# augustgw/early-exit-transformer

Hardware: AMD Instinct MI355X
Metric: mel-frames/sec encoder forward (all exits) + summed per-exit CTC loss, d_model=256 12-layer (higher is better)
Workload: dtype fp16x3 (hi/lo-split fp16 MFMA operands, three products per GEMM, fp32 accumulate; v_mfma_f32_16x16x32_f16); 1 GPU; early_conformer ctc 12-layer d_model=256 (6 exits x 2), batch 64/GPU, mel [80 x 1027] -> T'=256, log-normal synthetic mel, random-init weights (BASELINE.json configs[1]); global_batch=64, mel_frames=1027, parallelism=dp1 (utterance-batch shards), precision_mode=f16x3

## Files before the change

### early_exit_transformer_amd/csrc/ctc.hip

```cpp
#include <limits.h>

#include "eec_kernels.h"

namespace eec {

constexpr int kCtcPerLane = 8;
constexpr int kCtcEmpty = -(1 << 20);
constexpr float kCtcTiny = 7.52316385e-37f;
constexpr float kCtcRedo = -1.f;
__host__ __device__ inline int ctc_watch_slack(int Tq) {
  int lg = 0;
  while (((long long)Tq * 2048) >> lg) ++lg;
  return 120 - 26 - lg;
}

#define EEC_DPP_F(old, src, ctrl) \
  __builtin_bit_cast(float, __builtin_amdgcn_update_dpp(__builtin_bit_cast(int, (float)(old)), __builtin_bit_cast(int, (float)(src)), ctrl, 0xf, 0xf, false))
#define EEC_DPP_I(old, src, ctrl) __builtin_amdgcn_update_dpp((int)(old), (int)(src), ctrl, 0xf, 0xf, false)

__device__ __forceinline__ size_t ctc_store_index(int lat, int Tq, int P, int t, int k, int lane) {
  return (((size_t)lat * Tq + t) * (P + 1) + k) * 64 + lane;
}

template <int P, bool STORE>
__global__ __launch_bounds__(64) void ctc_alpha_kernel(const float* __restrict__ logp, const long long* __restrict__ targets,
                                                       const long long* __restrict__ target_len, int B, int Tq, int V,
                                                       int S, int blank, float* __restrict__ nll, float* __restrict__ astore) {
  const int lat = blockIdx.x, b = lat % B, lane = threadIdx.x;
  const float* lp = logp + (size_t)lat * Tq * V;
  const long long len_raw = target_len[b];
  bool bad = len_raw < 0 || len_raw > (long long)S;
  const int len = bad ? 0 : (int)len_raw;
  const int L = 2 * len + 1;
  int label[P];
  bool skip_ok[P], live[P];
#pragma unroll
  for (int i = 0; i < P; ++i) {
    const int s = lane * P + i;
    label[i] = blank;
    skip_ok[i] = false;
    live[i] = s < L;
    if (s < L && (s & 1)) {
      const int k = s >> 1;
      const long long lab = targets[(size_t)b * S + k];
      if (lab < 0 || lab >= (long long)V) bad = true;
      label[i] = (lab < 0 || lab >= (long long)V) ? blank : (int)lab;
      skip_ok[i] = k > 0 && lab != targets[(size_t)b * S + k - 1];
    }
  }
  bad = __any((int)bad) != 0;
  float livef[P];
#pragma unroll
  for (int i = 0; i < P; ++i) {
    livef[i] = live[i] ? 1.f : 0.f;
    asm volatile("" : "+v"(label[i]));
  }
  float alpha[P], lim[P];
  int ex = kCtcEmpty;
  static_assert(P % 2 == 0, "a lane's first state must be a blank");
  int eloss = kCtcEmpty;
#pragma unroll
  for (int i = 0; i < P; ++i) {
    const int s = lane * P + i;
    const float l0 = lp[label[i]];
    alpha[i] = (s < 2 && s < L) ? __expf(l0) : 0.f;
    eloss = ((s < 2 && s < L) & (l0 > -INFINITY) & (alpha[i] < kCtcTiny)) ? 0 : eloss;
    lim[i] = live[i] ? -INFINITY : INFINITY;
  }
  if (lane == 0) ex = 0;
  auto store = [&](int t) {
    if constexpr (STORE) {
#pragma unroll
      for (int i = 0; i < P; ++i) astore[ctc_store_index(lat, Tq, P, t, i, lane)] = alpha[i];
      astore[ctc_store_index(lat, Tq, P, t, P, lane)] = __builtin_bit_cast(float, ex);
    }
  };
  store(0);
  constexpr int kCtcAhead = P <= 4 ? 16 : 8;
  float emit[kCtcAhead][P];
#pragma unroll
  for (int d = 0; d < kCtcAhead; ++d)
#pragma unroll
    for (int i = 0; i < P; ++i) emit[d][i] = lp[(size_t)min(1 + d, Tq - 1) * V + label[i]];
  auto step = [&](const float (&em)[P], bool renorm) {
    float up1 = EEC_DPP_F(0.f, alpha[P - 1], 0x138);
    float up2 = EEC_DPP_F(0.f, alpha[P - 2], 0x138);
    const int ex_up = EEC_DPP_I(ex, ex, 0x138);
    const int ec = max(ex, ex_up);
    const int d_own = max(ex - ec, -200), d_up = max(ex_up - ec, -200);
    const float up1s = ldexpf(up1, d_up), up2s = ldexpf(up2, d_up);
    bool lost = (up1 > 0.f) & (up1s < kCtcTiny);
    up1 = up1s;
    up2 = up2s;
    float cur[P];
#pragma unroll
    for (int i = 0; i < P; ++i) {
      cur[i] = ldexpf(alpha[i], d_own);
      lost |= (alpha[i] > 0.f) & (cur[i] < kCtcTiny);
    }
    ex = ec;
#pragma unroll
    for (int i = 0; i < P; ++i) {
      const float p1 = i >= 1 ? cur[i - 1] : up1;
      const float p2 = i >= 2 ? cur[i - 2] : (i == 1 ? up1 : up2);
      const float sum = cur[i] + p1 + (skip_ok[i] ? p2 : 0.f);
      alpha[i] = sum * (__expf(em[i]) * livef[i]);
      lost |= (sum > 0.f) & (alpha[i] < kCtcTiny) & (em[i] > lim[i]);
    }
    eloss = lost ? max(eloss, ec) : eloss;
    if (renorm) {
      float m = alpha[0];
#pragma unroll
      for (int i = 1; i < P; ++i) m = fmaxf(m, alpha[i]);
      const bool any = m > 0.f;
      const int e = any ? (int)((__builtin_bit_cast(unsigned, m) >> 23) & 0xffu) - 127 : 0;
#pragma unroll
      for (int i = 0; i < P; ++i) alpha[i] = ldexpf(alpha[i], -e);
      ex = any ? ex + e : kCtcEmpty;
    }
  };
  int t0 = 1;
  for (; t0 + kCtcAhead <= Tq; t0 += kCtcAhead) {
#pragma unroll
    for (int d = 0; d < kCtcAhead; ++d) {
      step(emit[d], (d & 1) != 0);
      store(t0 + d);
      const int tn = min(t0 + d + kCtcAhead, Tq - 1);
#pragma unroll
      for (int i = 0; i < P; ++i) emit[d][i] = lp[(size_t)tn * V + label[i]];
    }
  }
#pragma unroll
  for (int d = 0; d < kCtcAhead; ++d)
    if (t0 + d < Tq) {
      step(emit[d], (d & 1) != 0);
      store(t0 + d);
    }
  float tail = 0.f;
#pragma unroll
  for (int i = 0; i < P; ++i) {
    const int s = lane * P + i;
    if (s == L - 1 || s == L - 2) tail += alpha[i];
  }
  bad = bad || __any((int)(tail != tail)) != 0;
  const int e_lane = tail > 0.f ? ex : kCtcEmpty;
  const int e_max = (int)wave_max((float)e_lane);
  const float total = wave_sum(tail > 0.f ? ldexpf(tail, max(e_lane - e_max, -200)) : 0.f);
  const int e_tot = total > 0.f ? e_max + (int)((__builtin_bit_cast(unsigned, total) >> 23) & 0xffu) - 127 : 2 * kCtcEmpty;
  const bool redo = __any((int)(eloss > kCtcEmpty && eloss > e_tot + ctc_watch_slack(Tq))) != 0;
  if (lane == 0)
    nll[lat] = (bad || total != total) ? __builtin_nanf("")
               : redo                  ? -INFINITY
               : (total > 0.f)         ? -(logf(total) + (float)e_max * 0.6931471805599453f)
                                       : INFINITY;
  if constexpr (STORE) {
    if (lane == 0) {
      float* pinfo = astore + ctc_store_index(gridDim.x, Tq, P, 0, 0, 0) + 2 * (size_t)lat;
      pinfo[0] = (bad || total != total) ? __builtin_nanf("") : redo ? kCtcRedo : total;
      pinfo[1] = __builtin_bit_cast(float, e_max);
    }
  }
}

template <int P>
__global__ __launch_bounds__(64) void ctc_beta_kernel(const float* __restrict__ logp, const long long* __restrict__ targets,
                                                      const long long* __restrict__ target_len, int B, int Tq, int V,
                                                      int S, int blank, const float* __restrict__ nll, float* __restrict__ astore) {
  const int lat = blockIdx.x, b = lat % B, lane = threadIdx.x;
  const float* lp = logp + (size_t)lat * Tq * V;
  float* pinfo = astore + ctc_store_index(gridDim.x, Tq, P, 0, 0, 0) + 2 * (size_t)lat;
  if (pinfo[0] < 0.f) return;
  const long long len_raw = target_len[b];
  const int len = (len_raw < 0 || len_raw > (long long)S) ? 0 : (int)len_raw;
  const int L = 2 * len + 1;
  int label[P];
  bool skip_ok[P];
  float livef[P], lim[P];
  bool redo = false;
#pragma unroll
  for (int i = 0; i < P; ++i) {
    const int s = lane * P + i;
    label[i] = blank;
    skip_ok[i] = false;
    livef[i] = s < L ? 1.f : 0.f;
    lim[i] = s < L ? -INFINITY : INFINITY;
    if (s < L && (s & 1)) {
      const int k = s >> 1;
      const long long lab = targets[(size_t)b * S + k];
      label[i] = (lab < 0 || lab >= (long long)V) ? blank : (int)lab;
      skip_ok[i] = k > 0 && lab != targets[(size_t)b * S + k - 1];
    }
    asm volatile("" : "+v"(label[i]));
  }
  bool skip_dn[P];
  {
    const int n0 = EEC_DPP_I(0, (int)skip_ok[0], 0x130), n1 = EEC_DPP_I(0, (int)skip_ok[1], 0x130);
#pragma unroll
    for (int i = 0; i < P; ++i) skip_dn[i] = i + 2 < P ? skip_ok[i + 2] : ((i + 2 - P == 0 ? n0 : n1) != 0);
  }
  const float ptot = pinfo[0];
  const bool usable = ptot > 0.f && ptot < INFINITY;
  const int ishift = usable ? -__builtin_bit_cast(int, pinfo[1]) : 0;
  const float fscale = usable ? 1.0f / ptot : 0.f;
  const int e_ptot = (int)((__builtin_bit_cast(unsigned, ptot) >> 23) & 0xffu) - 127;
  const int e_harm = usable ? -ishift + e_ptot + ctc_watch_slack(Tq) : INT_MAX;
  const int sh_harm = 120 - 26 - 2 + e_ptot;
  float beta[P];
  int eb = kCtcEmpty;
  bool any0 = false;
#pragma unroll
  for (int i = 0; i < P; ++i) {
    const int s = lane * P + i;
    beta[i] = (s < L && (s == L - 1 || s == L - 2)) ? 1.f : 0.f;
    any0 = any0 || beta[i] != 0.f;
  }
  if (any0) eb = 0;
  constexpr int kAhead = P <= 4 ? 8 : 4;
  float emit[kAhead][P], al[kAhead][P + 1];
  auto fetch = [&](int slot, int t) {
    const int tc = max(t, 0);
#pragma unroll
    for (int i = 0; i < P; ++i) emit[slot][i] = lp[(size_t)tc * V + label[i]];
#pragma unroll
    for (int k = 0; k <= P; ++k) al[slot][k] = astore[ctc_store_index(lat, Tq, P, tc, k, lane)];
  };
#pragma unroll
  for (int d = 0; d < kAhead; ++d) fetch(d, Tq - 1 - d);
  auto step = [&](int slot, int t, bool renorm) {
    const int ea = __builtin_bit_cast(int, al[slot][P]);
    const int sh = max(min(ea + eb + ishift, 126), -300);
#pragma unroll
    for (int i = 0; i < P; ++i) {
      const float ab = al[slot][i] * beta[i];
      redo |= (al[slot][i] > 0.f) & (beta[i] > 0.f) & (ab < kCtcTiny) & (sh > sh_harm);
      astore[ctc_store_index(lat, Tq, P, t, i, lane)] = ldexpf(ab * fscale, sh) * livef[i];
    }
    float bw[P];
    bool lost = false;
#pragma unroll
    for (int i = 0; i < P; ++i) {
      bw[i] = beta[i] * (__expf(emit[slot][i]) * livef[i]);
      lost |= (beta[i] > 0.f) & (bw[i] < kCtcTiny) & (emit[slot][i] > lim[i]);
    }
    float dn1 = EEC_DPP_F(0.f, bw[0], 0x130);
    float dn2 = EEC_DPP_F(0.f, bw[1], 0x130);
    const int eb_dn = EEC_DPP_I(kCtcEmpty, eb, 0x130);
    const int ec = max(eb, eb_dn);
    const int d_own = max(eb - ec, -200), d_dn = max(eb_dn - ec, -200);
    const float dn1s = ldexpf(dn1, d_dn), dn2s = ldexpf(dn2, d_dn);
    lost |= ((dn1 > 0.f) & (dn1s < kCtcTiny)) | ((dn2 > 0.f) & (dn2s < kCtcTiny));
    dn1 = dn1s;
    dn2 = dn2s;
#pragma unroll
    for (int i = 0; i < P; ++i) {
      const float sh_own = ldexpf(bw[i], d_own);
      lost |= (bw[i] > 0.f) & (sh_own < kCtcTiny);
      bw[i] = sh_own;
    }
    eb = ec;
    redo |= lost & (ec > e_harm);
#pragma unroll
    for (int i = 0; i < P; ++i) {
      const float n1 = i + 1 < P ? bw[i + 1 < P ? i + 1 : 0] : dn1;
      const float n2 = i + 2 < P ? bw[i + 2 < P ? i + 2 : 0] : (i + 2 - P == 0 ? dn1 : dn2);
      beta[i] = bw[i] + n1 + (skip_dn[i] ? n2 : 0.f);
    }
    if (renorm) {
      float m = beta[0];
#pragma unroll
      for (int i = 1; i < P; ++i) m = fmaxf(m, beta[i]);
      const bool any = m > 0.f;
      const int e = any ? (int)((__builtin_bit_cast(unsigned, m) >> 23) & 0xffu) - 127 : 0;
#pragma unroll
      for (int i = 0; i < P; ++i) beta[i] = ldexpf(beta[i], -e);
      eb = any ? eb + e : kCtcEmpty;
    }
  };
  int t = Tq - 1;
  for (; t - kAhead + 1 >= 0; t -= kAhead) {
#pragma unroll
    for (int d = 0; d < kAhead; ++d) {
      step(d, t - d, (d & 1) != 0);
      fetch(d, t - d - kAhead);
    }
  }
#pragma unroll
  for (int d = 0; d < kAhead; ++d)
    if (t - d >= 0) step(d, t - d, (d & 1) != 0);
  if (usable && __any((int)redo) != 0 && lane == 0) pinfo[0] = kCtcRedo;
}

template <int P>
__global__ __launch_bounds__(256) void ctc_grad_kernel(const float* __restrict__ logp, const long long* __restrict__ targets,
                                                       const long long* __restrict__ target_len, int B, int Tq, int V, int S,
                                                       int blank, const float* __restrict__ nll, const float* __restrict__ astore,
                                                       const float* __restrict__ grad_loss, int n_rows, float* __restrict__ dlogp) {
  __shared__ float bins_all[4][256];
  const int lane = threadIdx.x & 63, w = threadIdx.x >> 6;
  const int row = blockIdx.x * 4 + w;
  float* bins = bins_all[w];
  const bool row_ok = row < n_rows;
  const int lat = row_ok ? row / Tq : 0, t = row_ok ? row - lat * Tq : 0, b = lat % B, e = lat / B;
  *(float4*)(bins + lane * 4) = make_float4(0.f, 0.f, 0.f, 0.f);
  __syncthreads();
  const long long len_raw = target_len[b];
  const int len = (len_raw < 0 || len_raw > (long long)S) ? 0 : (int)len_raw;
  const int L = 2 * len + 1;
  if (row_ok) {
#pragma unroll
    for (int i = 0; i < P; ++i) {
      const int s = lane * P + i;
      if (s < L) {
        int lab = blank;
        if (s & 1) {
          const long long lr = targets[(size_t)b * S + (s >> 1)];
          lab = (lr < 0 || lr >= (long long)V) ? blank : (int)lr;
        }
        atomicAdd(&bins[lab], astore[ctc_store_index(lat, Tq, P, t, i, lane)]);
      }
    }
  }
  __syncthreads();
  if (!row_ok) return;
  const float nl = nll[lat];
  float gs = grad_loss[e] / ((float)B * (float)(len > 0 ? len : 1));
  if (nl != nl) gs = nl;
  else if (!(nl < INFINITY)) gs = 0.f;
  const int c0 = lane * 4;
  if (c0 < V) {
    const size_t off = ((size_t)lat * Tq + t) * V + c0;
    const float4 l = *(const float4*)(logp + off);
    const float4 g = *(const float4*)(bins + c0);
    float4 o;
    o.x = gs * (__expf(l.x) - g.x), o.y = gs * (__expf(l.y) - g.y), o.z = gs * (__expf(l.z) - g.z), o.w = gs * (__expf(l.w) - g.w);
    if (gs == 0.f) o = make_float4(0.f, 0.f, 0.f, 0.f);
    *(float4*)(dlogp + off) = o;
  }
}

constexpr int kCtcWideEmpty = -(1 << 30);

__device__ __forceinline__ void ctc_wide_exp(float l, float& pm, int& k) {
  const float hi = l * 1.44269502f;
  const float lo = fmaf(l, 1.44269502f, -hi) + l * 1.92596299e-8f;
  const float kf = floorf(hi);
  const bool zero = !(l > -3.0e4f);
  pm = zero ? 0.f : exp2f((hi - kf) + lo);
  k = zero ? 0 : (int)kf;
}
__device__ __forceinline__ void ctc_wide_norm(float v, int base, float& m, int& e) {
  const int ex = (int)((__builtin_bit_cast(unsigned, v) >> 23) & 0xffu) - 127;
  const bool any = v > 0.f;
  m = any ? ldexpf(v, -ex) : 0.f;
  e = any ? base + ex : kCtcWideEmpty;
}
__device__ __forceinline__ float ctc_wide_add3(float m0, int e0, float m1, int e1, float m2, int e2, int& ec) {
  ec = max(e0, max(e1, e2));
  return ldexpf(m0, max(e0 - ec, -64)) + ldexpf(m1, max(e1 - ec, -64)) + ldexpf(m2, max(e2 - ec, -64));
}

template <int P, bool GRAD>
__global__ __launch_bounds__(64) void ctc_wide_kernel(const float* __restrict__ logp, const long long* __restrict__ targets,
                                                      const long long* __restrict__ target_len, int B, int Tq, int V, int S,
                                                      int blank, float* __restrict__ nll, float* __restrict__ astore) {
  const int lat = blockIdx.x, b = lat % B, lane = threadIdx.x;
  if constexpr (GRAD) {
    if (!(astore[ctc_store_index(gridDim.x, Tq, P, 0, 0, 0) + 2 * (size_t)lat] < 0.f)) return;
  } else {
    if (!(nll[lat] == -INFINITY)) return;
  }
  const float* lp = logp + (size_t)lat * Tq * V;
  int* estore = GRAD ? (int*)(astore + ctc_store_index(gridDim.x, Tq, P, 0, 0, 0) + 2 * (size_t)gridDim.x) : nullptr;
  const long long len_raw = target_len[b];
  const int len = (len_raw < 0 || len_raw > (long long)S) ? 0 : (int)len_raw;
  const int L = 2 * len + 1;
  int label[P];
  bool skip_ok[P], live[P];
#pragma unroll
  for (int i = 0; i < P; ++i) {
    const int s = lane * P + i;
    label[i] = blank;
    skip_ok[i] = false;
    live[i] = s < L;
    if (s < L && (s & 1)) {
      const int k = s >> 1;
      const long long lab = targets[(size_t)b * S + k];
      label[i] = (lab < 0 || lab >= (long long)V) ? blank : (int)lab;
      skip_ok[i] = k > 0 && lab != targets[(size_t)b * S + k - 1];
    }
  }
  float am[P];
  int ae[P];
#pragma unroll
  for (int i = 0; i < P; ++i) {
    const int s = lane * P + i;
    float pm;
    int k;
    ctc_wide_exp(lp[label[i]], pm, k);
    ctc_wide_norm((s < 2 && s < L) ? pm : 0.f, k, am[i], ae[i]);
  }
  auto store = [&](int t) {
    if constexpr (GRAD) {
#pragma unroll
      for (int i = 0; i < P; ++i) {
        astore[ctc_store_index(lat, Tq, P, t, i, lane)] = am[i];
        estore[(((size_t)lat * Tq + t) * P + i) * 64 + lane] = ae[i];
      }
    }
  };
  store(0);
  constexpr int kAhead = 4;
  float emit[kAhead][P];
#pragma unroll
  for (int d = 0; d < kAhead; ++d)
#pragma unroll
    for (int i = 0; i < P; ++i) emit[d][i] = lp[(size_t)min(1 + d, Tq - 1) * V + label[i]];
  for (int t0 = 1; t0 < Tq; t0 += kAhead)
#pragma unroll
  for (int d = 0; d < kAhead; ++d) {
    const int t = t0 + d;
    if (t >= Tq) break;
    const float u1m = EEC_DPP_F(0.f, am[P - 1], 0x138), u2m = EEC_DPP_F(0.f, am[P - 2], 0x138);
    const int u1e = EEC_DPP_I(kCtcWideEmpty, ae[P - 1], 0x138), u2e = EEC_DPP_I(kCtcWideEmpty, ae[P - 2], 0x138);
    float nm[P];
    int ne[P];
#pragma unroll
    for (int i = 0; i < P; ++i) {
      const float p1m = i >= 1 ? am[i >= 1 ? i - 1 : 0] : u1m;
      const int p1e = i >= 1 ? ae[i >= 1 ? i - 1 : 0] : u1e;
      float p2m = i >= 2 ? am[i >= 2 ? i - 2 : 0] : (i == 1 ? u1m : u2m);
      int p2e = i >= 2 ? ae[i >= 2 ? i - 2 : 0] : (i == 1 ? u1e : u2e);
      if (!skip_ok[i]) p2m = 0.f, p2e = kCtcWideEmpty;
      float pm;
      int k, ec;
      ctc_wide_exp(emit[d][i], pm, k);
      const float sum = ctc_wide_add3(am[i], ae[i], p1m, p1e, p2m, p2e, ec);
      ctc_wide_norm(live[i] ? sum * pm : 0.f, ec + k, nm[i], ne[i]);
    }
#pragma unroll
    for (int i = 0; i < P; ++i) {
      am[i] = nm[i], ae[i] = ne[i];
      emit[d][i] = lp[(size_t)min(t + kAhead, Tq - 1) * V + label[i]];
    }
    store(t);
  }
  float tm = 0.f;
  int te = kCtcWideEmpty;
#pragma unroll
  for (int i = 0; i < P; ++i) {
    const int s = lane * P + i;
    if (s == L - 1 || s == L - 2) {
      int ec;
      tm = ctc_wide_add3(tm, te, am[i], ae[i], 0.f, kCtcWideEmpty, ec);
      te = tm > 0.f ? ec : kCtcWideEmpty;
    }
  }
  int e_max = te;
#pragma unroll
  for (int off = 32; off >= 1; off >>= 1) e_max = max(e_max, __shfl_xor(e_max, off, 64));
  float total = ldexpf(tm, max(te - e_max, -64));
#pragma unroll
  for (int off = 32; off >= 1; off >>= 1) total += __shfl_xor(total, off, 64);
  float mt;
  int et;
  ctc_wide_norm(total, e_max, mt, et);
  if constexpr (!GRAD) {
    if (lane == 0) nll[lat] = total > 0.f ? -(logf(mt) + (float)et * 0.6931471805599453f) : INFINITY;
    return;
  } else {
    if (!(total > 0.f)) return;
    bool skip_dn[P];
    {
      int n0 = __shfl_down((int)skip_ok[0], 1, 64), n1 = __shfl_down((int)skip_ok[1], 1, 64);
      if (lane == 63) n0 = n1 = 0;
#pragma unroll
      for (int i = 0; i < P; ++i) skip_dn[i] = i + 2 < P ? skip_ok[i + 2 < P ? i + 2 : 0] : ((i + 2 - P == 0 ? n0 : n1) != 0);
    }
    const float inv = 1.0f / mt;
    float bm[P];
    int be[P];
#pragma unroll
    for (int i = 0; i < P; ++i) {
      const int s = lane * P + i;
      const bool last = s < L && (s == L - 1 || s == L - 2);
      bm[i] = last ? 1.f : 0.f;
      be[i] = last ? 0 : kCtcWideEmpty;
    }
    for (int t = Tq - 1; t >= 0; --t) {
      float wm[P];
      int we[P];
#pragma unroll
      for (int i = 0; i < P; ++i) {
        const size_t ia = ctc_store_index(lat, Tq, P, t, i, lane);
        const float a_m = astore[ia];
        const int a_e = estore[(((size_t)lat * Tq + t) * P + i) * 64 + lane];
        const bool nz = a_m > 0.f && bm[i] > 0.f;
        const int sh = nz ? min(max(a_e + be[i] - et, -200), 126) : 0;
        astore[ia] = nz ? ldexpf(a_m * bm[i] * inv, sh) : 0.f;
        float pm;
        int k;
        ctc_wide_exp(lp[(size_t)t * V + label[i]], pm, k);
        ctc_wide_norm(live[i] ? bm[i] * pm : 0.f, be[i] + k, wm[i], we[i]);
      }
      float d1m = __shfl_down(wm[0], 1, 64), d2m = __shfl_down(wm[1], 1, 64);
      int d1e = __shfl_down(we[0], 1, 64), d2e = __shfl_down(we[1], 1, 64);
      if (lane == 63) d1m = d2m = 0.f, d1e = d2e = kCtcWideEmpty;
#pragma unroll
      for (int i = 0; i < P; ++i) {
        const float n1m = i + 1 < P ? wm[i + 1 < P ? i + 1 : 0] : d1m;
        const int n1e = i + 1 < P ? we[i + 1 < P ? i + 1 : 0] : d1e;
        float n2m = i + 2 < P ? wm[i + 2 < P ? i + 2 : 0] : (i + 2 - P == 0 ? d1m : d2m);
        int n2e = i + 2 < P ? we[i + 2 < P ? i + 2 : 0] : (i + 2 - P == 0 ? d1e : d2e);
        if (!skip_dn[i]) n2m = 0.f, n2e = kCtcWideEmpty;
        int ec;
        const float sum = ctc_wide_add3(wm[i], we[i], n1m, n1e, n2m, n2e, ec);
        ctc_wide_norm(sum, ec, bm[i], be[i]);
      }
    }
  }
}

int ctc_states_per_lane(int S) {
  if (2 * S + 1 <= 64 * 2) return 2;
  if (2 * S + 1 <= 64 * 4) return 4;
  if (2 * S + 1 <= 64 * kCtcPerLane) return kCtcPerLane;
  return 0;
}

size_t ctc_store_floats(int E, int B, int Tq, int S) {
  const int P = ctc_states_per_lane(S);
  return P ? (size_t)E * B * Tq * (P + 1) * 64 + 2 * (size_t)E * B + (size_t)E * B * Tq * P * 64 : 0;
}

hipError_t launch_ctc_backward(const float* logp, const long long* targets, const long long* target_len, int E, int B, int Tq,
                               int V, int S, int blank, const float* nll, float* astore, const float* grad_loss, float* dlogp,
                               hipStream_t st) {
  const int P = ctc_states_per_lane(S), n_rows = E * B * Tq;
  if (!P || V > 256 || V % 4) return hipErrorInvalidValue;
#define EEC_CTC_BWD(P_)                                                                                                      \
  hipLaunchKernelGGL(ctc_beta_kernel<P_>, dim3(E * B), dim3(64), 0, st, logp, targets, target_len, B, Tq, V, S, blank, nll,  \
                     astore);                                                                                               \
  hipLaunchKernelGGL((ctc_wide_kernel<P_, true>), dim3(E * B), dim3(64), 0, st, logp, targets, target_len, B, Tq, V, S,      \
                     blank, (float*)nullptr, astore);                                                                        \
  hipLaunchKernelGGL(ctc_grad_kernel<P_>, dim3((n_rows + 3) / 4), dim3(256), 0, st, logp, targets, target_len, B, Tq, V, S,  \
                     blank, nll, astore, grad_loss, n_rows, dlogp);
  if (P == 2) {
    EEC_CTC_BWD(2)
  } else if (P == 4) {
    EEC_CTC_BWD(4)
  } else {
    EEC_CTC_BWD(kCtcPerLane)
  }
#undef EEC_CTC_BWD
  return hipGetLastError();
}

__global__ void ctc_reduce_kernel(const float* nll, const long long* target_len, int B, float* out) {
  const int e = blockIdx.x, lane = threadIdx.x;
  float s = 0.f;
  for (int b0 = 0; b0 < B; b0 += 64) {
    const int b = b0 + lane;
    float term = 0.f;
    if (b < B) {
      float v = nll[e * B + b];
      if (isinf(v)) v = 0.f;
      const long long l = target_len[b] > 0 ? target_len[b] : 1;
      term = v / (float)l;
    }
    const int n = min(64, B - b0);
    for (int i = 0; i < n; ++i) s += __shfl(term, i, 64);
  }
  if (lane == 0) out[e] = s / (float)B;
}

hipError_t launch_ctc_loss(const float* logp, const long long* targets, const long long* target_len, int E, int B, int Tq,
                           int V, int S, int blank, float* nll, float* out, float* astore, hipStream_t st) {
  const int P = ctc_states_per_lane(S);
  if (!P) return hipErrorInvalidValue;
#define EEC_CTC_FWD(P_)                                                                                                        \
  if (astore)                                                                                                                  \
    hipLaunchKernelGGL((ctc_alpha_kernel<P_, true>), dim3(E * B), dim3(64), 0, st, logp, targets, target_len, B, Tq, V, S,     \
                       blank, nll, astore);                                                                                    \
  else                                                                                                                         \
    hipLaunchKernelGGL((ctc_alpha_kernel<P_, false>), dim3(E * B), dim3(64), 0, st, logp, targets, target_len, B, Tq, V, S,    \
                       blank, nll, astore);                                                                                    \
  hipLaunchKernelGGL((ctc_wide_kernel<P_, false>), dim3(E * B), dim3(64), 0, st, logp, targets, target_len, B, Tq, V, S,       \
                     blank, nll, astore);
  if (P == 2) {
    EEC_CTC_FWD(2)
  } else if (P == 4) {
    EEC_CTC_FWD(4)
  } else {
    EEC_CTC_FWD(kCtcPerLane)
  }
#undef EEC_CTC_FWD
  hipError_t e = hipGetLastError();
  if (e != hipSuccess) return e;
  hipLaunchKernelGGL(ctc_reduce_kernel, dim3(E), dim3(64), 0, st, nll, target_len, B, out);
  return hipGetLastError();
}

__global__ __launch_bounds__(256) void logsoftmax_bwd_kernel(const float* __restrict__ logp, const float* __restrict__ g, int M, int V,
                                                             float* __restrict__ dlogits) {
  const int lane = threadIdx.x & 63, row = blockIdx.x * 4 + (threadIdx.x >> 6);
  if (row >= M) return;
  const int c0 = lane * 4;
  float4 gv = make_float4(0.f, 0.f, 0.f, 0.f), lv = gv;
  if (c0 < V) {
    gv = *(const float4*)(g + (size_t)row * V + c0);
    lv = *(const float4*)(logp + (size_t)row * V + c0);
  }
  const float sum = wave_sum(gv.x + gv.y + gv.z + gv.w);
  if (c0 < V)
    *(float4*)(dlogits + (size_t)row * V + c0) = make_float4(gv.x - __expf(lv.x) * sum, gv.y - __expf(lv.y) * sum,
                                                             gv.z - __expf(lv.z) * sum, gv.w - __expf(lv.w) * sum);
}

hipError_t launch_logsoftmax_backward(const float* logp, const float* g, int M, int V, float* dlogits, hipStream_t st) {
  if (V > 256 || V % 4) return hipErrorInvalidValue;
  hipLaunchKernelGGL(logsoftmax_bwd_kernel, dim3((M + 3) / 4), dim3(256), 0, st, logp, g, M, V, dlogits);
  return hipGetLastError();
}

}
```

Baseline: 19.11 million mel-frames/s.

## Add bidirectional split-time CTC loss kernel for forward-only loss path

The forward-only path no longer runs the alpha kernel. It now uses a new two-wave kernel: one wave runs alpha over the first half of time, the other runs beta backward over the second half, and the halves meet through shared memory. The new kernel uses wide mantissa/exponent arithmetic, which removes the separate fallback pass. This is meant to halve the serial time-step chain of the CTC recursion. The cost is two waves per utterance, plus extra exp and normalisation arithmetic at every step.

```diff
diff --git a/early_exit_transformer_amd/csrc/ctc.hip b/early_exit_transformer_amd/csrc/ctc.hip
--- a/early_exit_transformer_amd/csrc/ctc.hip
+++ b/early_exit_transformer_amd/csrc/ctc.hip
@@ -22,7 +22,7 @@
   return (((size_t)lat * Tq + t) * (P + 1) + k) * 64 + lane;
 }
 
-template <int P, bool STORE>
+template <int P>
 __global__ __launch_bounds__(64) void ctc_alpha_kernel(const float* __restrict__ logp, const long long* __restrict__ targets,
                                                        const long long* __restrict__ target_len, int B, int Tq, int V,
                                                        int S, int blank, float* __restrict__ nll, float* __restrict__ astore) {
@@ -69,11 +69,9 @@
   }
   if (lane == 0) ex = 0;
   auto store = [&](int t) {
-    if constexpr (STORE) {
-#pragma unroll
-      for (int i = 0; i < P; ++i) astore[ctc_store_index(lat, Tq, P, t, i, lane)] = alpha[i];
-      astore[ctc_store_index(lat, Tq, P, t, P, lane)] = __builtin_bit_cast(float, ex);
-    }
+#pragma unroll
+    for (int i = 0; i < P; ++i) astore[ctc_store_index(lat, Tq, P, t, i, lane)] = alpha[i];
+    astore[ctc_store_index(lat, Tq, P, t, P, lane)] = __builtin_bit_cast(float, ex);
   };
   store(0);
   constexpr int kCtcAhead = P <= 4 ? 16 : 8;
@@ -153,12 +151,10 @@
                : redo                  ? -INFINITY
                : (total > 0.f)         ? -(logf(total) + (float)e_max * 0.6931471805599453f)
                                        : INFINITY;
-  if constexpr (STORE) {
-    if (lane == 0) {
-      float* pinfo = astore + ctc_store_index(gridDim.x, Tq, P, 0, 0, 0) + 2 * (size_t)lat;
-      pinfo[0] = (bad || total != total) ? __builtin_nanf("") : redo ? kCtcRedo : total;
-      pinfo[1] = __builtin_bit_cast(float, e_max);
-    }
+  if (lane == 0) {
+    float* pinfo = astore + ctc_store_index(gridDim.x, Tq, P, 0, 0, 0) + 2 * (size_t)lat;
+    pinfo[0] = (bad || total != total) ? __builtin_nanf("") : redo ? kCtcRedo : total;
+    pinfo[1] = __builtin_bit_cast(float, e_max);
   }
 }
 
@@ -359,18 +355,14 @@
   return ldexpf(m0, max(e0 - ec, -64)) + ldexpf(m1, max(e1 - ec, -64)) + ldexpf(m2, max(e2 - ec, -64));
 }
 
-template <int P, bool GRAD>
+template <int P>
 __global__ __launch_bounds__(64) void ctc_wide_kernel(const float* __restrict__ logp, const long long* __restrict__ targets,
                                                       const long long* __restrict__ target_len, int B, int Tq, int V, int S,
                                                       int blank, float* __restrict__ nll, float* __restrict__ astore) {
   const int lat = blockIdx.x, b = lat % B, lane = threadIdx.x;
-  if constexpr (GRAD) {
-    if (!(astore[ctc_store_index(gridDim.x, Tq, P, 0, 0, 0) + 2 * (size_t)lat] < 0.f)) return;
-  } else {
-    if (!(nll[lat] == -INFINITY)) return;
-  }
+  if (!(astore[ctc_store_index(gridDim.x, Tq, P, 0, 0, 0) + 2 * (size_t)lat] < 0.f)) return;
   const float* lp = logp + (size_t)lat * Tq * V;
-  int* estore = GRAD ? (int*)(astore + ctc_store_index(gridDim.x, Tq, P, 0, 0, 0) + 2 * (size_t)gridDim.x) : nullptr;
+  int* estore = (int*)(astore + ctc_store_index(gridDim.x, Tq, P, 0, 0, 0) + 2 * (size_t)gridDim.x);
   const long long len_raw = target_len[b];
   const int len = (len_raw < 0 || len_raw > (long long)S) ? 0 : (int)len_raw;
   const int L = 2 * len + 1;
@@ -400,12 +392,10 @@
     ctc_wide_norm((s < 2 && s < L) ? pm : 0.f, k, am[i], ae[i]);
   }
   auto store = [&](int t) {
-    if constexpr (GRAD) {
-#pragma unroll
-      for (int i = 0; i < P; ++i) {
-        astore[ctc_store_index(lat, Tq, P, t, i, lane)] = am[i];
-        estore[(((size_t)lat * Tq + t) * P + i) * 64 + lane] = ae[i];
-      }
+#pragma unroll
+    for (int i = 0; i < P; ++i) {
+      astore[ctc_store_index(lat, Tq, P, t, i, lane)] = am[i];
+      estore[(((size_t)lat * Tq + t) * P + i) * 64 + lane] = ae[i];
     }
   };
   store(0);
@@ -464,60 +454,235 @@
   float mt;
   int et;
   ctc_wide_norm(total, e_max, mt, et);
-  if constexpr (!GRAD) {
-    if (lane == 0) nll[lat] = total > 0.f ? -(logf(mt) + (float)et * 0.6931471805599453f) : INFINITY;
+  if (!(total > 0.f)) return;
+  bool skip_dn[P];
+  {
+    int n0 = __shfl_down((int)skip_ok[0], 1, 64), n1 = __shfl_down((int)skip_ok[1], 1, 64);
+    if (lane == 63) n0 = n1 = 0;
+#pragma unroll
+    for (int i = 0; i < P; ++i) skip_dn[i] = i + 2 < P ? skip_ok[i + 2 < P ? i + 2 : 0] : ((i + 2 - P == 0 ? n0 : n1) != 0);
+  }
+  const float inv = 1.0f / mt;
+  float bm[P];
+  int be[P];
+#pragma unroll
+  for (int i = 0; i < P; ++i) {
+    const int s = lane * P + i;
+    const bool last = s < L && (s == L - 1 || s == L - 2);
+    bm[i] = last ? 1.f : 0.f;
+    be[i] = last ? 0 : kCtcWideEmpty;
+  }
+  for (int t = Tq - 1; t >= 0; --t) {
+    float wm[P];
+    int we[P];
+#pragma unroll
+    for (int i = 0; i < P; ++i) {
+      const size_t ia = ctc_store_index(lat, Tq, P, t, i, lane);
+      const float a_m = astore[ia];
+      const int a_e = estore[(((size_t)lat * Tq + t) * P + i) * 64 + lane];
+      const bool nz = a_m > 0.f && bm[i] > 0.f;
+      const int sh = nz ? min(max(a_e + be[i] - et, -200), 126) : 0;
+      astore[ia] = nz ? ldexpf(a_m * bm[i] * inv, sh) : 0.f;
+      float pm;
+      int k;
+      ctc_wide_exp(lp[(size_t)t * V + label[i]], pm, k);
+      ctc_wide_norm(live[i] ? bm[i] * pm : 0.f, be[i] + k, wm[i], we[i]);
+    }
+    float d1m = __shfl_down(wm[0], 1, 64), d2m = __shfl_down(wm[1], 1, 64);
+    int d1e = __shfl_down(we[0], 1, 64), d2e = __shfl_down(we[1], 1, 64);
+    if (lane == 63) d1m = d2m = 0.f, d1e = d2e = kCtcWideEmpty;
+#pragma unroll
+    for (int i = 0; i < P; ++i) {
+      const float n1m = i + 1 < P ? wm[i + 1 < P ? i + 1 : 0] : d1m;
+      const int n1e = i + 1 < P ? we[i + 1 < P ? i + 1 : 0] : d1e;
+      float n2m = i + 2 < P ? wm[i + 2 < P ? i + 2 : 0] : (i + 2 - P == 0 ? d1m : d2m);
+      int n2e = i + 2 < P ? we[i + 2 < P ? i + 2 : 0] : (i + 2 - P == 0 ? d1e : d2e);
+      if (!skip_dn[i]) n2m = 0.f, n2e = kCtcWideEmpty;
+      int ec;
+      const float sum = ctc_wide_add3(wm[i], we[i], n1m, n1e, n2m, n2e, ec);
+      ctc_wide_norm(sum, ec, bm[i], be[i]);
+    }
+  }
+}
+
+__device__ __forceinline__ void ctc_loss_exp(float l, float& pm, int& k) {
+  const float hi = l * 1.44269502f;
+  const float lo = fmaf(l, 1.44269502f, -hi) + l * 1.92596299e-8f;
+  const float kf = floorf(hi);
+  pm = l <= -3.0e4f ? 0.f : __builtin_amdgcn_exp2f((hi - kf) + lo);
+  k = l > -3.0e4f ? (int)kf : 0;
+}
+__device__ __forceinline__ void ctc_loss_norm(float v, int base, float& m, int& e) {
+  const int ex = (int)((__builtin_bit_cast(unsigned, v) >> 23) & 0xffu) - 127;
+  m = ldexpf(v, -ex);
+  e = v != 0.f ? base + ex : kCtcWideEmpty;
+}
+
+template <int P, bool DOWN>
+__device__ __forceinline__ void ctc_loss_sums(const float (&xm)[P], const int (&xe)[P], const bool (&skip)[P], float (&sum)[P],
+                                              int (&ec)[P]) {
+  constexpr int ctrl = DOWN ? 0x130 : 0x138;
+  const float u1m = EEC_DPP_F(0.f, xm[DOWN ? 0 : P - 1], ctrl), u2m = EEC_DPP_F(0.f, xm[DOWN ? 1 : P - 2], ctrl);
+  const int u1e = EEC_DPP_I(kCtcWideEmpty, xe[DOWN ? 0 : P - 1], ctrl), u2e = EEC_DPP_I(kCtcWideEmpty, xe[DOWN ? 1 : P - 2], ctrl);
+#pragma unroll
+  for (int i = 0; i < P; ++i) {
+    const int d1 = DOWN ? i + 1 : i - 1, d2 = DOWN ? i + 2 : i - 2;
+    const bool in1 = d1 >= 0 && d1 < P, in2 = d2 >= 0 && d2 < P;
+    const bool far2 = DOWN ? d2 == P + 1 : d2 == -2;
+    const float n1m = in1 ? xm[in1 ? d1 : 0] : u1m;
+    const int n1e = in1 ? xe[in1 ? d1 : 0] : u1e;
+    float n2m = in2 ? xm[in2 ? d2 : 0] : (far2 ? u2m : u1m);
+    int n2e = in2 ? xe[in2 ? d2 : 0] : (far2 ? u2e : u1e);
+    if (!skip[i]) n2m = 0.f, n2e = kCtcWideEmpty;
+    sum[i] = ctc_wide_add3(xm[i], xe[i], n1m, n1e, n2m, n2e, ec[i]);
+  }
+}
+
+template <int P, bool DOWN>
+__device__ __forceinline__ void ctc_loss_walk(const float* __restrict__ lp, int V, const int (&label)[P], const bool (&skip)[P],
+                                              const bool (&live)[P], int t_first, int n, float (&xm)[P], int (&xe)[P]) {
+  if (n <= 0) return;
+  constexpr int kAhead = P <= 4 ? 16 : 8;
+  float emit[kAhead][P];
+  auto gather = [&](float (&em)[P], int j) {
+    const float* row = lp + (size_t)(DOWN ? t_first - min(j, n - 1) : t_first + min(j, n - 1)) * V;
+#pragma unroll
+    for (int i = 0; i < P; ++i) em[i] = *(const float*)((const char*)row + (unsigned)label[i]);
+  };
+#pragma unroll
+  for (int d = 0; d < kAhead; ++d) gather(emit[d], d);
+  auto step = [&](const float (&em)[P]) {
+    float sum[P];
+    int ec[P];
+    ctc_loss_sums<P, DOWN>(xm, xe, skip, sum, ec);
+#pragma unroll
+    for (int i = 0; i < P; ++i) {
+      float pm;
+      int k;
+      ctc_loss_exp(em[i], pm, k);
+      const bool keep = DOWN ? sum[i] != 0.f : live[i];
+      ctc_loss_norm(keep ? sum[i] * pm : 0.f, ec[i] + k, xm[i], xe[i]);
+    }
+  };
+  int j0 = 0;
+  for (; j0 + kAhead <= n; j0 += kAhead) {
+#pragma unroll
+    for (int d = 0; d < kAhead; ++d) {
+      step(emit[d]);
+      gather(emit[d], j0 + d + kAhead);
+    }
+  }
+#pragma unroll
+  for (int d = 0; d < kAhead; ++d)
+    if (j0 + d < n) step(emit[d]);
+}
+
+template <int P>
+__global__ __launch_bounds__(128) void ctc_loss_kernel(const float* __restrict__ logp, const long long* __restrict__ targets,
+                                                       const long long* __restrict__ target_len, int B, int Tq, int V, int S,
+                                                       int blank, int only_marked, float* __restrict__ nll) {
+  __shared__ float beta_m[P][64];
+  __shared__ int beta_e[P][64];
+  const int lat = blockIdx.x, b = lat % B, lane = threadIdx.x & 63;
+  const bool down = __builtin_amdgcn_readfirstlane((int)threadIdx.x >> 6) != 0;
+  if (only_marked && !(nll[lat] == -INFINITY)) return;
+  const float* lp = logp + (size_t)lat * Tq * V;
+  const long long len_raw = target_len[b];
+  bool bad = len_raw < 0 || len_raw > (long long)S;
+  const int len = bad ? 0 : (int)len_raw;
+  const int L = 2 * len + 1;
+  int label[P];
+  bool skip_ok[P], live[P], last[P];
+#pragma unroll
+  for (int i = 0; i < P; ++i) {
+    const int s = lane * P + i;
+    label[i] = blank;
+    skip_ok[i] = false;
+    live[i] = s < L;
+    last[i] = s < L && (s == L - 1 || s == L - 2);
+    if (s < L && (s & 1)) {
+      const int k = s >> 1;
+      const long long lab = targets[(size_t)b * S + k];
+      if (lab < 0 || lab >= (long long)V) bad = true;
+      label[i] = (lab < 0 || lab >= (long long)V) ? blank : (int)lab;
+      skip_ok[i] = k > 0 && lab != targets[(size_t)b * S + k - 1];
+    }
+  }
+  bad = __any((int)bad) != 0;
+  if (bad) {
+    if (threadIdx.x == 0) nll[lat] = __builtin_nanf("");
     return;
+  }
+#pragma unroll
+  for (int i = 0; i < P; ++i) {
+    label[i] *= (int)sizeof(float);
+    asm volatile("" : "+v"(label[i]));
+  }
+  static_assert(P % 2 == 0, "a lane's first state must be a blank");
+  auto at = [&](int t, int i) { return *(const float*)((const char*)(lp + (size_t)t * V) + (unsigned)label[i]); };
+  const int m = (Tq - 1) / 2;
+  float xm[P];
+  int xe[P];
+  if (!down) {
+#pragma unroll
+    for (int i = 0; i < P; ++i) {
+      const int s = lane * P + i;
+      float pm;
+      int k;
+      ctc_loss_exp(at(0, i), pm, k);
+      ctc_loss_norm((s < 2 && s < L) ? pm : 0.f, k, xm[i], xe[i]);
+    }
+    ctc_loss_walk<P, false>(lp, V, label, skip_ok, live, 1, m, xm, xe);
   } else {
-    if (!(total > 0.f)) return;
-    bool skip_dn[P];
-    {
-      int n0 = __shfl_down((int)skip_ok[0], 1, 64), n1 = __shfl_down((int)skip_ok[1], 1, 64);
-      if (lane == 63) n0 = n1 = 0;
+    if (Tq - 1 > m) {
+      bool skip_dn[P];
+      const int n0 = EEC_DPP_I(0, (int)skip_ok[0], 0x130), n1 = EEC_DPP_I(0, (int)skip_ok[1], 0x130);
 #pragma unroll
       for (int i = 0; i < P; ++i) skip_dn[i] = i + 2 < P ? skip_ok[i + 2 < P ? i + 2 : 0] : ((i + 2 - P == 0 ? n0 : n1) != 0);
-    }
-    const float inv = 1.0f / mt;
-    float bm[P];
-    int be[P];
-#pragma unroll
-    for (int i = 0; i < P; ++i) {
-      const int s = lane * P + i;
-      const bool last = s < L && (s == L - 1 || s == L - 2);
-      bm[i] = last ? 1.f : 0.f;
-      be[i] = last ? 0 : kCtcWideEmpty;
-    }
-    for (int t = Tq - 1; t >= 0; --t) {
-      float wm[P];
-      int we[P];
 #pragma unroll
       for (int i = 0; i < P; ++i) {
-        const size_t ia = ctc_store_index(lat, Tq, P, t, i, lane);
-        const float a_m = astore[ia];
-        const int a_e = estore[(((size_t)lat * Tq + t) * P + i) * 64 + lane];
-        const bool nz = a_m > 0.f && bm[i] > 0.f;
-        const int sh = nz ? min(max(a_e + be[i] - et, -200), 126) : 0;
-        astore[ia] = nz ? ldexpf(a_m * bm[i] * inv, sh) : 0.f;
         float pm;
         int k;
-        ctc_wide_exp(lp[(size_t)t * V + label[i]], pm, k);
-        ctc_wide_norm(live[i] ? bm[i] * pm : 0.f, be[i] + k, wm[i], we[i]);
+        ctc_loss_exp(at(Tq - 1, i), pm, k);
+        ctc_loss_norm(last[i] ? pm : 0.f, k, xm[i], xe[i]);
       }
-      float d1m = __shfl_down(wm[0], 1, 64), d2m = __shfl_down(wm[1], 1, 64);
-      int d1e = __shfl_down(we[0], 1, 64), d2e = __shfl_down(we[1], 1, 64);
-      if (lane == 63) d1m = d2m = 0.f, d1e = d2e = kCtcWideEmpty;
-#pragma unroll
-      for (int i = 0; i < P; ++i) {
-        const float n1m = i + 1 < P ? wm[i + 1 < P ? i + 1 : 0] : d1m;
-        const int n1e = i + 1 < P ? we[i + 1 < P ? i + 1 : 0] : d1e;
-        float n2m = i + 2 < P ? wm[i + 2 < P ? i + 2 : 0] : (i + 2 - P == 0 ? d1m : d2m);
-        int n2e = i + 2 < P ? we[i + 2 < P ? i + 2 : 0] : (i + 2 - P == 0 ? d1e : d2e);
-        if (!skip_dn[i]) n2m = 0.f, n2e = kCtcWideEmpty;
-        int ec;
-        const float sum = ctc_wide_add3(wm[i], we[i], n1m, n1e, n2m, n2e, ec);
-        ctc_wide_norm(sum, ec, bm[i], be[i]);
-      }
-    }
-  }
+      ctc_loss_walk<P, true>(lp, V, label, skip_dn, live, Tq - 2, Tq - 2 - m, xm, xe);
+      float sum[P];
+      int ec[P];
+      ctc_loss_sums<P, true>(xm, xe, skip_dn, sum, ec);
+#pragma unroll
+      for (int i = 0; i < P; ++i) ctc_loss_norm(sum[i], ec[i], xm[i], xe[i]);
+    } else {
+#pragma unroll
+      for (int i = 0; i < P; ++i) xm[i] = last[i] ? 1.f : 0.f, xe[i] = last[i] ? 0 : kCtcWideEmpty;
+    }
+#pragma unroll
+    for (int i = 0; i < P; ++i) beta_m[i][lane] = xm[i], beta_e[i][lane] = xe[i];
+  }
+  __syncthreads();
+  if (down) return;
+  float tm[P];
+  int te[P], e_lane = kCtcWideEmpty;
+#pragma unroll
+  for (int i = 0; i < P; ++i) {
+    const float bm = beta_m[i][lane];
+    tm[i] = bm == 0.f ? 0.f : xm[i] * bm;
+    te[i] = tm[i] != 0.f ? max(xe[i], kCtcWideEmpty / 2) + max(beta_e[i][lane], kCtcWideEmpty / 2) : kCtcWideEmpty;
+    e_lane = max(e_lane, te[i]);
+  }
+  float tl = 0.f;
+#pragma unroll
+  for (int i = 0; i < P; ++i) tl += ldexpf(tm[i], max(te[i] - e_lane, -64));
+  int e_max = e_lane;
+#pragma unroll
+  for (int off = 32; off >= 1; off >>= 1) e_max = max(e_max, __shfl_xor(e_max, off, 64));
+  float total = ldexpf(tl, max(e_lane - e_max, -64));
+#pragma unroll
+  for (int off = 32; off >= 1; off >>= 1) total += __shfl_xor(total, off, 64);
+  float mt;
+  int et;
+  ctc_loss_norm(total, e_max, mt, et);
+  if (lane == 0) nll[lat] = total != 0.f ? -(logf(mt) + (float)et * 0.6931471805599453f) : INFINITY;
 }
 
 int ctc_states_per_lane(int S) {
@@ -540,8 +705,8 @@
 #define EEC_CTC_BWD(P_)                                                                                                      \
   hipLaunchKernelGGL(ctc_beta_kernel<P_>, dim3(E * B), dim3(64), 0, st, logp, targets, target_len, B, Tq, V, S, blank, nll,  \
                      astore);                                                                                               \
-  hipLaunchKernelGGL((ctc_wide_kernel<P_, true>), dim3(E * B), dim3(64), 0, st, logp, targets, target_len, B, Tq, V, S,      \
-                     blank, (float*)nullptr, astore);                                                                        \
+  hipLaunchKernelGGL(ctc_wide_kernel<P_>, dim3(E * B), dim3(64), 0, st, logp, targets, target_len, B, Tq, V, S, blank,       \
+                     (float*)nullptr, astore);                                                                               \
   hipLaunchKernelGGL(ctc_grad_kernel<P_>, dim3((n_rows + 3) / 4), dim3(256), 0, st, logp, targets, target_len, B, Tq, V, S,  \
                      blank, nll, astore, grad_loss, n_rows, dlogp);
   if (P == 2) {
@@ -577,15 +742,12 @@
                            int V, int S, int blank, float* nll, float* out, float* astore, hipStream_t st) {
   const int P = ctc_states_per_lane(S);
   if (!P) return hipErrorInvalidValue;
-#define EEC_CTC_FWD(P_)                                                                                                        \
-  if (astore)                                                                                                                  \
-    hipLaunchKernelGGL((ctc_alpha_kernel<P_, true>), dim3(E * B), dim3(64), 0, st, logp, targets, target_len, B, Tq, V, S,     \
-                       blank, nll, astore);                                                                                    \
-  else                                                                                                                         \
-    hipLaunchKernelGGL((ctc_alpha_kernel<P_, false>), dim3(E * B), dim3(64), 0, st, logp, targets, target_len, B, Tq, V, S,    \
-                       blank, nll, astore);                                                                                    \
-  hipLaunchKernelGGL((ctc_wide_kernel<P_, false>), dim3(E * B), dim3(64), 0, st, logp, targets, target_len, B, Tq, V, S,       \
-                     blank, nll, astore);
+#define EEC_CTC_FWD(P_)                                                                                                      \
+  if (astore)                                                                                                                \
+    hipLaunchKernelGGL(ctc_alpha_kernel<P_>, dim3(E * B), dim3(64), 0, st, logp, targets, target_len, B, Tq, V, S, blank,    \
+                       nll, astore);                                                                                         \
+  hipLaunchKernelGGL(ctc_loss_kernel<P_>, dim3(E * B), dim3(128), 0, st, logp, targets, target_len, B, Tq, V, S, blank,      \
+                     astore ? 1 : 0, nll);
   if (P == 2) {
     EEC_CTC_FWD(2)
   } else if (P == 4) {
```

Result: faster. 19.61 million mel-frames/s, median of 6 (+2.6%).
